# ZHKKKe/PixelSSL

Hardware: NVIDIA H100
Metric: images/sec DeepLab-v2-R101 MT 513x513 bs16 (higher is better)
Workload: dtype f16x3 (fp16 pairs, fp32 accumulate)

## Files before the change

include/pixelssl_b200.h:

```cpp
#ifndef PIXELSSL_B200_H
#define PIXELSSL_B200_H

#include <stdint.h>

#ifdef __cplusplus
extern "C" {
#endif

#define PXL_ERR_BAD_ARG   (-1)
#define PXL_ERR_UNSUPPORTED (-2)

int pxl_abi_version(void);
int64_t pxl_launch_count(void);
void pxl_reset_launch_count(void);

int64_t pxl_mse_workspace_bytes(void);
int pxl_mse_consistency(const float* s, const float* t, int64_t n, float loss_scale,
                        float* loss_out, float* grad_s, void* workspace, void* stream);
int pxl_mse_consistency_bwd(const float* s, const float* t, int64_t n, float loss_scale,
                            const float* upstream, float* grad_s, void* stream);

int pxl_ce2d(const float* logits, const float* labels, int n, int C, int64_t HW, int ignore_index,
             float* per_sample, float* grad_logits, const float* upstream, float upstream_const,
             void* stream);
// ... 69 lines not shown
} pxl_conv_geom;
#define PXL_MAX_TAPS 64
int pxl_conv_nhwc(const pxl_conv_geom* geom_host, const int* taps_dydx_host ,
                  const float* in, const float* w, const float* bias ,
                  float* out, void* stream);
int pxl_conv_wgrad_nhwc(const pxl_conv_geom* geom_host, const int* taps_dydx_host,
                        const float* in, const float* dy, float* dw, void* stream);
typedef struct {
    int w_ntaps;
    const int* widx_host;
    int out_mul, out_offy, out_offx, out_H, out_W;
    double* bn_stats;
    float out_scale;
    const float* out_scale_dev;
    int out_accumulate;
} pxl_conv_tc_ext;
int pxl_conv_tc_launch_ex(const pxl_conv_geom* geom_host, const int* taps_dydx_host, const pxl_conv_tc_ext* ext_host,
                          const float* in_hi, const float* in_lo, const float* w_hi, const float* w_lo,
                          const float* bias, float* out, void* stream);
int pxl_conv_wgrad_tc_launch(const pxl_conv_geom* geom_host, const int* taps_dydx_host, const float* in_hi,
                             const float* in_lo, const float* dy_hi, const float* dy_lo, float* dw,
                             void* stream);
int pxl_conv_h16_launch(const pxl_conv_geom* geom_host, const int* taps_dydx_host, const pxl_conv_tc_ext* ext_host,
                        const void* in_hi, const void* in_lo, const void* w_hi, const void* w_lo,
                        const float* bias, float* out, void* stream);
int pxl_conv_wgrad_h16_launch(const pxl_conv_geom* geom_host, const int* taps_dydx_host, const void* in_hi,
                              const void* in_lo, const void* dy_hi, const void* dy_lo, float* dw, float out_scale,
                              const float* out_scale_dev, void* stream);
int pxl_h16_split(const float* x, void* hi, void* lo, int64_t n, float scale, float* slot, int target_log2,
                  void* stream);
int pxl_h16_absmax(const float* x, int64_t n, float* slot, void* stream);
int pxl_h16_status(void);
int pxl_h16_status_sites(int* out4_host);
int pxl_h16_reset_status(void);
int pxl_split_tf32(const float* x, float* hi, float* lo, int64_t n, void* stream);
int pxl_conv_tc_status(void);
int pxl_conv_transpose_weights(const float* w, float* wt, int Cout, int T, int Cin, void* stream);
int pxl_conv_transpose_weights_batched(const float* src_base, float* dst_base, const int64_t* table, int n,
                                       int64_t total_tiles, void* stream);
int pxl_bias_grad(const float* dy, int64_t rows, int Cout, int ldo, float* dbias, int accumulate,
                  void* stream);

int pxl_stem_conv7x7s2(const float* img_planar, const float* w, float* out, int N, int H, int W,
                       int OH, int OW, void* stream);
int pxl_stem_conv7x7s2_wgrad(const float* img_planar, const float* dy, float* dw, int N, int H, int W,
                             int OH, int OW, void* stream);
int pxl_stem_im2col(const float* img_planar, float* cols, int N, int H, int W, int OH, int OW, void* stream);
int pxl_stem3x3s2_im2col(const float* img_planar, float* cols, int N, int H, int W, int OH, int OW, void* stream);

int pxl_sgd_ema(float* p, const float* g, float* buf, float* teacher, int64_t n, float lr,
                float momentum, float weight_decay, float ema_d, int first_step, void* stream);
// ... 102 lines not shown
```

pixelssl_b200/_lib.py:

```python
import ctypes
import os
import re

_HERE = os.path.dirname(os.path.abspath(__file__))
LIB_PATH = os.path.join(_HERE, 'lib', 'libpixelssl_b200.so')
HEADER_PATH = os.path.join(os.path.dirname(_HERE), 'include', 'pixelssl_b200.h')

c_void_p, c_int, c_int64, c_float, c_double = (ctypes.c_void_p, ctypes.c_int, ctypes.c_int64,
                                               ctypes.c_float, ctypes.c_double)
_SCALARS = {'int': c_int, 'int64_t': c_int64, 'float': c_float, 'double': c_double}


class ConvGeom(ctypes.Structure):
    _fields_ = [('N', c_int), ('H', c_int), ('W', c_int), ('Cin', c_int),
                ('OH', c_int), ('OW', c_int), ('Cout', c_int), ('ldo', c_int),
                ('mul', c_int), ('div', c_int), ('ntaps', c_int), ('precision', c_int)]


class ConvTcExt(ctypes.Structure):
    _fields_ = [('w_ntaps', c_int), ('widx_host', ctypes.POINTER(c_int)), ('out_mul', c_int),
                ('out_offy', c_int), ('out_offx', c_int), ('out_H', c_int), ('out_W', c_int),
                ('bn_stats', c_void_p), ('out_scale', c_float), ('out_scale_dev', c_void_p), ('out_accumulate', c_int)]


def header_code(path=HEADER_PATH):
    text = re.sub(r'/\*.*?\*/', ' ', open(path).read(), flags=re.S)
    return re.sub(r'^\s*#.*$', ' ', text, flags=re.M)


def ctype_of(decl, name, returned=False):
    if '*' in decl:
        return c_void_p
    words = [w for w in decl.split() if w != 'const']
    if returned and words == ['void']:
        return None
    t = ' '.join(words if returned else words[:-1])
    if t not in _SCALARS:
# ... 66 lines not shown
```

pixelssl_b200/csrc/common.cuh:

```cuda
#pragma once
#include <cuda_runtime.h>
#include <stdint.h>
#include "../../include/pixelssl_b200.h"

#define PXL_NUM_SMS 132

extern "C" void pxl_count_launch_(int n);
extern "C" int* pxl_h16_sat_counter(void);

#define PXL_WS_WGRAD 0
#define PXL_WS_BIAS 1
#define PXL_WS_CE 2
#define PXL_WS_CPS 3
#define PXL_WS_UNIMATCH 4
#define PXL_WS_STRONG_AUG 5
#define PXL_WS_OHEM 6
#define PXL_WS_DEPTHWISE 7
#define PXL_WS_PURPOSES 8
#define PXL_WS_STREAMS 8
extern "C" void* pxl_workspace_(int purpose, void* stream, size_t bytes, int* rc);

#define PXL_CHECK_LAUNCH()                                   \
    do {                                                     \
        pxl_count_launch_(1);                                \
        cudaError_t e__ = cudaPeekAtLastError();             \
        if (e__ != cudaSuccess) return (int)e__;             \
    } while (0)

static inline int64_t pxl_cdiv(int64_t a, int64_t b) { return (a + b - 1) / b; }

#define PXL_PDL_SYNC()                                                   \
    do {                                                                 \
        asm volatile("griddepcontrol.launch_dependents;" ::: "memory");  \
// ... 54 lines not shown
```

pixelssl_b200/csrc/conv_tc.cu:

```cuda
#include "common.cuh"
#include <cuda.h>
#include <cstdlib>
#include <type_traits>

typedef CUresult (*EncodeTiledFn)(CUtensorMap*, CUtensorMapDataType, cuuint32_t, void*, const cuuint64_t*,
                                  const cuuint64_t*, const cuuint32_t*, const cuuint32_t*, CUtensorMapInterleave,
                                  CUtensorMapSwizzle, CUtensorMapL2promotion, CUtensorMapFloatOOBfill);
static EncodeTiledFn get_encode() {
    static EncodeTiledFn fn = nullptr;
    if (!fn) {
        void* p = nullptr;
        cudaDriverEntryPointQueryResult q;
        if (cudaGetDriverEntryPoint("cuTensorMapEncodeTiled", &p, cudaEnableDefault, &q) == cudaSuccess &&
            q == cudaDriverEntryPointSuccess)
            fn = (EncodeTiledFn)p;
    }
    return fn;
}

static int make_act_map(CUtensorMap* m, const void* base, int C, int W, int H, int N, int bw, int bh, int estride = 1, int f16 = 0) {
    EncodeTiledFn enc = get_encode();
    if (!enc) return PXL_ERR_UNSUPPORTED;
    const cuuint64_t eb = f16 ? 2 : 4;
    cuuint64_t dims[4] = {(cuuint64_t)C, (cuuint64_t)W, (cuuint64_t)H, (cuuint64_t)N};
// ... 80 lines not shown
    uint64_t d = 0;
    d |= (uint64_t)((smem_addr & 0x3FFFF) >> 4);
    d |= (uint64_t)((lbo_bytes >> 4) & 0x3FFF) << 16;
    d |= (uint64_t)(1024 >> 4) << 32;
    d |= (uint64_t)1 << 62;
    return d;
}
__device__ __forceinline__ void wg_arrive() { asm volatile("wgmma.fence.sync.aligned;" ::: "memory"); }
__device__ __forceinline__ void wg_commit() { asm volatile("wgmma.commit_group.sync.aligned;" ::: "memory"); }
__device__ __forceinline__ void wg_wait0() { asm volatile("wgmma.wait_group.sync.aligned 0;" ::: "memory"); }
template <int R>
__device__ __forceinline__ void fence_regs(float (&d)[R]) {
#pragma unroll
    for (int i = 0; i < R; ++i) asm volatile("" : "+f"(d[i])::"memory");
}

template <int N, int KIND>
__device__ __forceinline__ void wgmma_op(float (&d)[N / 2], uint64_t da, uint64_t db, int scale_d);
template <> __device__ __forceinline__ void wgmma_op<32, 0>(float (&d)[16], uint64_t da, uint64_t db, int scale_d) {
    asm volatile(
        "{\n\t.reg .pred p;\n\tsetp.ne.b32 p, %18, 0;\n\t"
        "wgmma.mma_async.sync.aligned.m64n32k8.f32.tf32.tf32 {%0, %1, %2, %3, %4, %5, %6, %7, %8, %9, %10, %11, %12, %13, %14, %15}, %16, %17, p, 1, 1;\n\t}"
        : "+f"(d[0]), "+f"(d[1]), "+f"(d[2]), "+f"(d[3]), "+f"(d[4]), "+f"(d[5]), "+f"(d[6]), "+f"(d[7]), "+f"(d[8]), "+f"(d[9]), "+f"(d[10]), "+f"(d[11]), "+f"(d[12]), "+f"(d[13]), "+f"(d[14]), "+f"(d[15])
        : "l"(da), "l"(db), "r"(scale_d));
}
template <> __device__ __forceinline__ void wgmma_op<64, 0>(float (&d)[32], uint64_t da, uint64_t db, int scale_d) {
    asm volatile(
        "{\n\t.reg .pred p;\n\tsetp.ne.b32 p, %34, 0;\n\t"
        "wgmma.mma_async.sync.aligned.m64n64k8.f32.tf32.tf32 {%0, %1, %2, %3, %4, %5, %6, %7, %8, %9, %10, %11, %12, %13, %14, %15, %16, %17, %18, %19, %20, %21, %22, %23, %24, %25, %26, %27, %28, %29, %30, %31}, %32, %33, p, 1, 1;\n\t}"
        : "+f"(d[0]), "+f"(d[1]), "+f"(d[2]), "+f"(d[3]), "+f"(d[4]), "+f"(d[5]), "+f"(d[6]), "+f"(d[7]), "+f"(d[8]), "+f"(d[9]), "+f"(d[10]), "+f"(d[11]), "+f"(d[12]), "+f"(d[13]), "+f"(d[14]), "+f"(d[15]), "+f"(d[16]), "+f"(d[17]), "+f"(d[18]), "+f"(d[19]), "+f"(d[20]), "+f"(d[21]), "+f"(d[22]), "+f"(d[23]), "+f"(d[24]), "+f"(d[25]), "+f"(d[26]), "+f"(d[27]), "+f"(d[28]), "+f"(d[29]), "+f"(d[30]), "+f"(d[31])
// ... 69 lines not shown
    return h;
}

struct TcParams {
    int Cin, Cout, ldo, ntaps, kchunks;
    int N, OH, OW;
    int BW, BH, tilesW, tilesH;
    int stages, nsplit;
    int a_inkernel;
    int in_mul;
    int out_mul, out_offy, out_offx, outH, outW;
    int ntilesN, pix_tiles, total_tiles;
    int kc;
    float out_scale;
    int out_acc;
    short dy[PXL_MAX_TAPS], dx[PXL_MAX_TAPS], widx[PXL_MAX_TAPS];
};

#define TC_A_BYTES (128 * 128)
#define TC_MAX_STAGES 8
#define TC_THREADS 384

__device__ __forceinline__ void tc_tile_coords(const TcParams& p, int tile, int bn, int& n0, int& w0, int& h0, int& n) {
    const int nt = tile / p.pix_tiles, pix = tile - nt * p.pix_tiles;
    const int tw = pix % p.tilesW, th = (pix / p.tilesW) % p.tilesH;
    n = pix / (p.tilesW * p.tilesH);
    w0 = tw * p.BW; h0 = th * p.BH; n0 = nt * bn;
}

template <int BN, int F16>
__global__ void __launch_bounds__(TC_THREADS, 1)
conv_wg_kernel(const __grid_constant__ CUtensorMap mapA, const __grid_constant__ CUtensorMap mapAlo,
               const __grid_constant__ CUtensorMap mapB, const __grid_constant__ CUtensorMap mapBlo,
               const TcParams p, const float* __restrict__ bias, float* __restrict__ out,
               double* __restrict__ stats, int* __restrict__ err_flag, const float* __restrict__ oscale_ptr) {
    extern __shared__ __align__(1024) uint8_t smem_raw[];
    __shared__ uint64_t full_bar[TC_MAX_STAGES], empty_bar[TC_MAX_STAGES];
    __shared__ float st_warp[2][8][BN];

    uint8_t* smem = (uint8_t*)(((uintptr_t)smem_raw + 1023) & ~(uintptr_t)1023);
    constexpr int B_BYTES = BN * 128;
    constexpr int PER_OP = TC_A_BYTES + B_BYTES;
    const int stage_bytes = PER_OP * (p.nsplit == 3 ? 2 : 1);
    const int iters = p.ntaps * p.kchunks;

    if (threadIdx.x == 0) {
        for (int s = 0; s < p.stages; ++s) { mbar_init(&full_bar[s], 1); mbar_init(&empty_bar[s], 256); }
        asm volatile("fence.mbarrier_init.release.cluster;" ::: "memory");
    }
    __syncthreads();
    PXL_PDL_SYNC();

    if (threadIdx.x < 128) {
        asm volatile("setmaxnreg.dec.sync.aligned.u32 40;" ::: "memory");
        if (threadIdx.x >= 32) return;
        uint32_t tx = (uint32_t)((p.BW * p.BH * 128 + B_BYTES) * (p.nsplit == 3 ? 2 : 1));
        if (p.a_inkernel) tx -= (uint32_t)(p.BW * p.BH * 128);
        uint32_t s = 0, ph = 0;
        bool ok = true;
        for (int tile = blockIdx.x; tile < p.total_tiles && ok; tile += gridDim.x) {
            int n0, w0, h0, n;
            tc_tile_coords(p, tile, BN, n0, w0, h0, n);
            int tap = 0, c0 = 0;
            for (int it = 0; it < iters; ++it) {
                ok = __all_sync(0xffffffffu, mbar_wait(&empty_bar[s], ph ^ 1u, err_flag, 1));
                if (!ok) break;
                uint8_t* sa = smem + (size_t)s * stage_bytes;
                const int ax = w0 * p.in_mul + p.dx[tap], ay = h0 * p.in_mul + p.dy[tap];
                const int bk = p.widx[tap] * p.Cin + c0;
                if (elect_one()) {
                    mbar_expect_tx(&full_bar[s], tx);
                    tma_load_4d(sa, &mapA, &full_bar[s], c0, ax, ay, n);
                    tma_load_2d(sa + TC_A_BYTES, &mapB, &full_bar[s], bk, n0);
                    if (p.nsplit == 3) {
                        if (!p.a_inkernel) tma_load_4d(sa + PER_OP, &mapAlo, &full_bar[s], c0, ax, ay, n);
                        tma_load_2d(sa + PER_OP + TC_A_BYTES, &mapBlo, &full_bar[s], bk, n0);
                    }
                }
                __syncwarp();
                c0 += p.kc; if (c0 >= p.Cin) { c0 = 0; ++tap; }
                if (++s == (uint32_t)p.stages) { s = 0; ph ^= 1u; }
            }
        }
        return;
    }

    asm volatile("setmaxnreg.inc.sync.aligned.u32 232;" ::: "memory");
    const int ct = threadIdx.x - 128;
    const int cw = ct >> 7, t = ct & 127;
    const int warp = t >> 5, lane = t & 31;
    const float osc = p.out_scale * (oscale_ptr ? __ldg(oscale_ptr) : 1.f);
    const uint32_t smem_base = smem_u32(smem);
    const bool split3 = p.nsplit == 3;
    float acc[BN / 2], part[BN / 2], corr[BN / 2];
    uint32_t s = 0, ph = 0;
    int st_n0 = -1;
    float st_s = 0.f, st_q = 0.f;
    bool ok = true;
    auto flush_stats = [&]() {
        if (st_n0 >= 0 && ct < BN && st_n0 + ct < p.Cout && (st_s != 0.f || st_q != 0.f)) {
            atomicAdd(stats + st_n0 + ct, (double)st_s);
            atomicAdd(stats + p.Cout + st_n0 + ct, (double)st_q);
        }
        st_s = 0.f; st_q = 0.f;
    };
    auto f16_tile = [&](auto split3_c) -> bool {
        constexpr bool S3 = decltype(split3_c)::value;
        uint32_t prev = 0;
        for (int it = 0; it < iters; ++it) {
            if (!__all_sync(0xffffffffu, mbar_wait(&full_bar[s], ph, err_flag, 2))) { wg_wait0(); return false; }
            const uint32_t sa32 = smem_base + s * (uint32_t)stage_bytes;
            const uint32_t arow = (uint32_t)cw * (TC_A_BYTES / 2);
            const uint64_t da = sw128_desc(sa32 + arow), db = sw128_desc(sa32 + TC_A_BYTES);
            const uint64_t dal = sw128_desc(sa32 + PER_OP + arow), dbl = sw128_desc(sa32 + PER_OP + TC_A_BYTES);
            wg_arrive();
            fence_regs(part);
            if (S3) fence_regs(corr);
#pragma unroll
            for (int k = 0; k < 2; ++k) wgmma_op<BN, 1>(part, da + 2 * k, db + 2 * k, k);
            wg_commit();
            if (S3) {
#pragma unroll
                for (int k = 0; k < 4; ++k) wgmma_op<BN, 1>(corr, dal + 2 * k, db + 2 * k, k);
#pragma unroll
                for (int k = 0; k < 4; ++k) wgmma_op<BN, 1>(corr, da + 2 * k, dbl + 2 * k, 1);
                wg_commit();
                asm volatile("wgmma.wait_group.sync.aligned 1;" ::: "memory");
                fence_regs(part);
#pragma unroll
                for (int i = 0; i < BN / 2; ++i) acc[i] += part[i];
                wg_arrive();
                fence_regs(part);
#pragma unroll
                for (int k = 2; k < 4; ++k) wgmma_op<BN, 1>(part, da + 2 * k, db + 2 * k, k - 2);
                wg_commit();
                wg_wait0();
                fence_regs(part);
                fence_regs(corr);
                mbar_arrive(&empty_bar[s]);
#pragma unroll
                for (int i = 0; i < BN / 2; ++i) acc[i] += part[i] + corr[i];
            } else {
                asm volatile("wgmma.wait_group.sync.aligned 1;" ::: "memory");
                fence_regs(corr);
                if (it > 0) {
                    mbar_arrive(&empty_bar[prev]);
#pragma unroll
                    for (int i = 0; i < BN / 2; ++i) acc[i] += corr[i];
                }
                wg_arrive();
                fence_regs(corr);
#pragma unroll
                for (int k = 2; k < 4; ++k) wgmma_op<BN, 1>(corr, da + 2 * k, db + 2 * k, k - 2);
                wg_commit();
                asm volatile("wgmma.wait_group.sync.aligned 1;" ::: "memory");
                fence_regs(part);
#pragma unroll
                for (int i = 0; i < BN / 2; ++i) acc[i] += part[i];
            }
            prev = s;
            if (++s == (uint32_t)p.stages) { s = 0; ph ^= 1u; }
        }
        if (!S3) {
            wg_wait0();
            fence_regs(corr);
            mbar_arrive(&empty_bar[prev]);
#pragma unroll
            for (int i = 0; i < BN / 2; ++i) acc[i] += corr[i];
        }
        return true;
    };
    for (int tile = blockIdx.x; tile < p.total_tiles && ok; tile += gridDim.x) {
        int n0, w0, h0, n;
        tc_tile_coords(p, tile, BN, n0, w0, h0, n);
        if (stats && n0 != st_n0) { flush_stats(); st_n0 = n0; }
#pragma unroll
        for (int i = 0; i < BN / 2; ++i) acc[i] = 0.f;
        if constexpr (F16 != 0) ok = split3 ? f16_tile(std::true_type{}) : f16_tile(std::false_type{});
        else for (int it = 0; it < iters; ++it) {
            ok = __all_sync(0xffffffffu, mbar_wait(&full_bar[s], ph, err_flag, 2));
            if (!ok) break;
            uint8_t* sa = smem + (size_t)s * stage_bytes;
            if (p.a_inkernel) {
                float4* a_hi = reinterpret_cast<float4*>(sa + cw * (TC_A_BYTES / 2));
                float4* a_lo = reinterpret_cast<float4*>(sa + PER_OP + cw * (TC_A_BYTES / 2));
#pragma unroll
                for (int c = 0; c < TC_A_BYTES / 2 / 16 / 128; ++c) {
                    float4 lo;
                    const float4 hi = tf32_split4(a_hi[t + c * 128], lo);
                    a_hi[t + c * 128] = hi;
                    a_lo[t + c * 128] = lo;
                }
                fence_async_smem();
                named_bar(2 + cw, 128);
// ... 24 lines not shown
            for (int k = 2; k < 4; ++k) wgmma_op<BN, F16>(part, da + 2 * k, db + 2 * k, k - 2);
            wg_commit();
            wg_wait0();
            fence_regs(part);
            fence_regs(corr);
            mbar_arrive(&empty_bar[s]);
            if (split3) {
#pragma unroll
                for (int i = 0; i < BN / 2; ++i) acc[i] += part[i] + corr[i];
            } else {
#pragma unroll
                for (int i = 0; i < BN / 2; ++i) acc[i] += part[i];
            }
            if (++s == (uint32_t)p.stages) { s = 0; ph ^= 1u; }
        }
        if (!ok) break;
        int64_t obase[2];
        bool valid[2];
#pragma unroll
        for (int h = 0; h < 2; ++h) {
            const int r = cw * 64 + warp * 16 + (lane >> 2) + 8 * h;
            const int hy = r / p.BW, wx = r - hy * p.BW;
            const int oy = h0 + hy, ox = w0 + wx;
            valid[h] = hy < p.BH && oy < p.OH && ox < p.OW;
            obase[h] = ((int64_t)(n * p.outH + oy * p.out_mul + p.out_offy) * p.outW + ox * p.out_mul + p.out_offx) * p.ldo;
        }
        const bool vec2 = (p.ldo & 1) == 0 && ((uintptr_t)out & 7) == 0;
#pragma unroll
        for (int j = 0; j < BN / 8; ++j) {
            const int cl = j * 8 + 2 * (lane & 3);
            const int col = n0 + cl;
            const bool c0ok = col < p.Cout, c1ok = col + 1 < p.Cout;
            const float b0 = (bias && c0ok) ? __ldg(bias + col) : 0.f, b1 = (bias && c1ok) ? __ldg(bias + col + 1) : 0.f;
            float v[2][2];
#pragma unroll
            for (int h = 0; h < 2; ++h) {
                v[h][0] = acc[j * 4 + 2 * h] * osc + b0;
                v[h][1] = acc[j * 4 + 2 * h + 1] * osc + b1;
                if (!valid[h]) continue;
                float* o = out + obase[h] + col;
                if (p.out_acc) {
                    if (c0ok) o[0] += v[h][0];
                    if (c1ok) o[1] += v[h][1];
                } else if (c1ok && vec2) {
                    *reinterpret_cast<float2*>(o) = make_float2(v[h][0], v[h][1]);
                } else {
                    if (c0ok) o[0] = v[h][0];
// ... 5 lines not shown
                float s1 = (valid[0] ? v[0][1] : 0.f) + (valid[1] ? v[1][1] : 0.f);
                float q0 = (valid[0] ? v[0][0] * v[0][0] : 0.f) + (valid[1] ? v[1][0] * v[1][0] : 0.f);
                float q1 = (valid[0] ? v[0][1] * v[0][1] : 0.f) + (valid[1] ? v[1][1] * v[1][1] : 0.f);
#pragma unroll
                for (int o = 4; o < 32; o <<= 1) {
                    s0 += __shfl_xor_sync(0xffffffffu, s0, o); s1 += __shfl_xor_sync(0xffffffffu, s1, o);
                    q0 += __shfl_xor_sync(0xffffffffu, q0, o); q1 += __shfl_xor_sync(0xffffffffu, q1, o);
                }
                if (lane < 4) {
                    const int slot = cw * 4 + warp;
                    st_warp[0][slot][cl] = s0; st_warp[0][slot][cl + 1] = s1;
                    st_warp[1][slot][cl] = q0; st_warp[1][slot][cl + 1] = q1;
                }
            }
        }
        if (stats) {
            named_bar(1, 256);
            if (ct < BN) {
#pragma unroll
                for (int w8 = 0; w8 < 8; ++w8) { st_s += st_warp[0][w8][ct]; st_q += st_warp[1][w8][ct]; }
            }
            named_bar(1, 256);
        }
    }
    if (stats && ok) flush_stats();
}

__global__ void __launch_bounds__(256)
split_tf32_kernel(const float4* __restrict__ x, float4* __restrict__ hi, float4* __restrict__ lo, int64_t n4) {
    const int64_t stride = (int64_t)gridDim.x * blockDim.x;
    for (int64_t i = (int64_t)blockIdx.x * blockDim.x + threadIdx.x; i < n4; i += stride) {
        float4 l;
        hi[i] = tf32_split4(__ldcs(x + i), l);
        lo[i] = l;
    }
}

// ... 34 lines not shown
        int bh = 128 / bw;
        if (bh < 1) break;
        if (bh > 256) bh = 256;
        const int64_t tiles = (int64_t)((OW + bw - 1) / bw) * ((OH + bh - 1) / bh);
        const double eff = (double)OH * OW / ((double)tiles * 128.0);
        if (eff > best + 1e-9) { best = eff; BW = bw; BH = bh; }
    }
}

template <int BN, int F16>
static int fwd_smem_limit() {
    static const int v = query_dyn_smem_limit(conv_wg_kernel<BN, F16>);
    return v;
}

template <int BN, int F16>
static int launch_fwd(const CUtensorMap& mA, const CUtensorMap& mAlo, const CUtensorMap& mB, const CUtensorMap& mBlo,
                      const TcParams& p, size_t smem, cudaStream_t st, const float* bias, float* out, double* stats,
                      const float* oscale_ptr) {
    static bool attr = false;
    if (!attr) {
        cudaError_t e = cudaFuncSetAttribute(conv_wg_kernel<BN, F16>, cudaFuncAttributeMaxDynamicSharedMemorySize, fwd_smem_limit<BN, F16>());
        if (e != cudaSuccess) return (int)e;
        attr = true;
    }
    const unsigned nblk = (unsigned)(p.total_tiles < PXL_NUM_SMS ? p.total_tiles : PXL_NUM_SMS);
    cudaError_t le = pxl_launch_pdl(conv_wg_kernel<BN, F16>, dim3(nblk), dim3(TC_THREADS), smem, st, mA, mAlo, mB, mBlo, p,
                                    bias, out, stats, g_err_flag, oscale_ptr);
    if (le != cudaSuccess) return (int)le;
    PXL_CHECK_LAUNCH();
    return 0;
}

static int conv_tc_launch_core(const pxl_conv_geom* g, const int* taps, const pxl_conv_tc_ext* ext,
                               const void* in_hi, const void* in_lo, const void* w_hi, const void* w_lo,
                               const float* bias, float* out, void* stream);

extern "C" int pxl_conv_tc_launch_ex(const pxl_conv_geom* g, const int* taps, const pxl_conv_tc_ext* ext,
                                     const float* in_hi, const float* in_lo, const float* w_hi, const float* w_lo,
                                     const float* bias, float* out, void* stream) {
    if (g && g->precision > 2) return PXL_ERR_BAD_ARG;
    return conv_tc_launch_core(g, taps, ext, in_hi, in_lo, w_hi, w_lo, bias, out, stream);
}

extern "C" int pxl_conv_h16_launch(const pxl_conv_geom* g, const int* taps, const pxl_conv_tc_ext* ext,
                                   const void* in_hi, const void* in_lo, const void* w_hi, const void* w_lo,
                                   const float* bias, float* out, void* stream) {
    if (!g || (g->precision != 3 && g->precision != 4)) return PXL_ERR_BAD_ARG;
    return conv_tc_launch_core(g, taps, ext, in_hi, in_lo, w_hi, w_lo, bias, out, stream);
}

// ... 6 lines not shown
    const int kc = f16 ? 64 : 32;
    if (g->Cin % kc != 0 || g->ntaps > PXL_MAX_TAPS) return PXL_ERR_UNSUPPORTED;
    const int wtaps = ext && ext->w_ntaps > 0 ? ext->w_ntaps : g->ntaps;
    const int nsplit = (g->precision == 2 || g->precision == 3) ? 3 : 1;
    if (nsplit == 3 && !w_lo) return PXL_ERR_BAD_ARG;
    if (f16 && nsplit == 3 && !in_lo) return PXL_ERR_BAD_ARG;
    const int a_inkernel = (!f16 && nsplit == 3 && !in_lo) ? 1 : 0;
    const int omul = (ext && ext->out_mul > 0) ? ext->out_mul : 1;
    const bool has_out_xform = ext && (omul != 1 || ext->out_offy != 0 || ext->out_offx != 0);
    bool flat = (g->ntaps == 1 && taps[0] == 0 && taps[1] == 0 && g->OH == g->H && g->OW == g->W && g->mul == 1 &&
                 !has_out_xform);
    TcParams p;
    p.Cin = g->Cin; p.Cout = g->Cout; p.ldo = g->ldo; p.ntaps = g->ntaps; p.kchunks = g->Cin / kc;
    p.nsplit = nsplit; p.a_inkernel = a_inkernel; p.kc = kc;
    p.out_scale = (ext && ext->out_scale != 0.f) ? ext->out_scale : 1.f;
    const float* oscale_ptr = ext ? ext->out_scale_dev : nullptr;
    for (int t = 0; t < g->ntaps; ++t) {
        p.dy[t] = (short)taps[2 * t]; p.dx[t] = (short)taps[2 * t + 1];
        p.widx[t] = (short)((ext && ext->widx_host) ? ext->widx_host[t] : t);
        if (p.widx[t] < 0 || p.widx[t] >= wtaps) return PXL_ERR_BAD_ARG;
    }
    p.in_mul = g->mul;
    p.out_mul = omul; p.out_offy = has_out_xform ? ext->out_offy : 0; p.out_offx = has_out_xform ? ext->out_offx : 0;
    int mapW, mapH, mapN;
    if (flat) {
        const int64_t M = (int64_t)g->N * g->H * g->W;
        if (M >= (1ll << 31)) return PXL_ERR_UNSUPPORTED;
        p.N = 1; p.OH = 1; p.OW = (int)M;
        mapW = (int)M; mapH = 1; mapN = 1;
        p.outH = 1; p.outW = (int)M;
// ... 8 lines not shown
    const int stage_bytes = (TC_A_BYTES + BN * 128) * (nsplit == 3 ? 2 : 1);
    p.tilesW = (p.OW + p.BW - 1) / p.BW; p.tilesH = (p.OH + p.BH - 1) / p.BH;
    p.pix_tiles = p.N * p.tilesH * p.tilesW;
    p.ntilesN = (g->Cout + BN - 1) / BN;
    const int64_t n_tiles = (int64_t)p.pix_tiles * p.ntilesN;
    if (n_tiles >= (1ll << 31)) return PXL_ERR_UNSUPPORTED;
    p.total_tiles = (int)n_tiles;
    const int smem_limit = f16 ? (BN == 128 ? fwd_smem_limit<128, 1>() : BN == 64 ? fwd_smem_limit<64, 1>() : fwd_smem_limit<32, 1>())
                               : (BN == 128 ? fwd_smem_limit<128, 0>() : BN == 64 ? fwd_smem_limit<64, 0>() : fwd_smem_limit<32, 0>());
    if (smem_limit <= 0) return PXL_ERR_UNSUPPORTED;
    p.stages = (smem_limit - 1024) / stage_bytes;
    if (p.stages > TC_MAX_STAGES) p.stages = TC_MAX_STAGES;
    if (p.stages < 2) return PXL_ERR_UNSUPPORTED;
    const size_t smem = (size_t)p.stages * stage_bytes + 1024;

    CUtensorMap mA, mAlo, mB, mBlo;
    int rc = make_act_map(&mA, in_hi, g->Cin, mapW, mapH, mapN, p.BW, p.BH, g->mul, f16);
    if (rc) return rc;
    rc = make_w_map(&mB, w_hi, (int64_t)wtaps * g->Cin, g->Cout, BN, f16);
    if (rc) return rc;
    if (nsplit == 3) {
        if (a_inkernel) mAlo = mA;
        else {
            rc = make_act_map(&mAlo, in_lo, g->Cin, mapW, mapH, mapN, p.BW, p.BH, g->mul, f16);
            if (rc) return rc;
        }
        rc = make_w_map(&mBlo, w_lo, (int64_t)wtaps * g->Cin, g->Cout, BN, f16);
        if (rc) return rc;
    } else {
        mAlo = mA; mBlo = mB;
    }
    p.out_acc = (ext && ext->out_accumulate) ? 1 : 0;
    if ((rc = ensure_err_flag())) return rc;
    cudaStream_t st = (cudaStream_t)stream;
    double* st_ptr = ext ? (double*)ext->bn_stats : nullptr;
    if (f16) {
        if (BN == 128) return launch_fwd<128, 1>(mA, mAlo, mB, mBlo, p, smem, st, bias, out, st_ptr, oscale_ptr);
        if (BN == 64) return launch_fwd<64, 1>(mA, mAlo, mB, mBlo, p, smem, st, bias, out, st_ptr, oscale_ptr);
        return launch_fwd<32, 1>(mA, mAlo, mB, mBlo, p, smem, st, bias, out, st_ptr, oscale_ptr);
    }
    if (BN == 128) return launch_fwd<128, 0>(mA, mAlo, mB, mBlo, p, smem, st, bias, out, st_ptr, oscale_ptr);
    if (BN == 64) return launch_fwd<64, 0>(mA, mAlo, mB, mBlo, p, smem, st, bias, out, st_ptr, oscale_ptr);
    return launch_fwd<32, 0>(mA, mAlo, mB, mBlo, p, smem, st, bias, out, st_ptr, oscale_ptr);
}

extern "C" int pxl_conv_tc_status(void) {
    if (!g_err_flag) return 0;
    int v = 0;
    if (cudaMemcpy(&v, g_err_flag, sizeof(int), cudaMemcpyDeviceToHost) != cudaSuccess) return -1;
    return v;
}

extern "C" int pxl_conv_tc_impl(const pxl_conv_geom* g, const int* taps, const float* in, const float* w,
                                const float* bias, float* out, void* stream) {
    if (!g) return PXL_ERR_BAD_ARG;
    if (g->precision == 2) return PXL_ERR_UNSUPPORTED;
    if (g->precision > 2) return PXL_ERR_BAD_ARG;
    return conv_tc_launch_core(g, taps, nullptr, in, nullptr, w, nullptr, bias, out, stream);
// ... 405 lines not shown
```

pixelssl_b200/ops.py:

```python
import ctypes
import functools
import math

import torch

from . import _lib
from ._lib import ConvGeom, ConvTcExt, call
from .nn.peer import MAX_VALUES as _PEER_MAX_VALUES

CL = torch.channels_last
PRECISION = {'fp32': 0, 'tf32': 1, 'tf32x3': 2, 'f16x3': 3, 'f16': 4}
H16_FALLBACK = {3: 2, 4: 1}
H16_ACT_SCALE = 16.0
H16_W_SCALE = 256.0
H16_GRAD_TARGET_LOG2 = 14
_conv_precision = 0


def set_conv_precision(name):
    global _conv_precision
    _conv_precision = PRECISION[name]


def get_conv_precision():
    return _conv_precision


def _p(t):
    return t.data_ptr() if t is not None else None


# ... 630 lines not shown

def _stride2_dgrad_classes(taps, ntaps):
    classes = []
    for py in (0, 1):
        for px in (0, 1):
            sub, widx = [], []
            for t in range(ntaps):
                dy, dx = taps[2 * t], taps[2 * t + 1]
                if (py + dy) % 2 == 0 and (px + dx) % 2 == 0:
                    sub += [(py + dy) // 2, (px + dx) // 2]
                    widx.append(t)
            classes.append((py, px, sub, widx))
    return classes


def conv_raw(x, w_packed, bias, taps, N, H, W, Cin, OH, OW, Cout, ldo, mul, div, out=None, precision=None, bn_stats=None,
             accumulate=False):
    ntaps = len(taps) // 2
    family, prec = conv_route('fwd', Cin, Cout, mul, div, _conv_precision if precision is None else precision)
    if family != 'h16' and (isinstance(x, H16) or isinstance(w_packed, H16)):
        raise ValueError('fp16-pair operands given for a shape the f16 wgmma kernel does not cover')
    if out is None:
        out = torch.empty((N, ldo, OH, OW), dtype=torch.float32, device=(x[0] if isinstance(x, tuple) else x).device,
                          memory_format=CL)
        if ldo != Cout:
            out.zero_()
    if family == 'ffma':
        if isinstance(x, tuple):
            x = x[0] + x[1]
        if isinstance(w_packed, tuple):
            w_packed = w_packed[0] + w_packed[1]
        geom = ConvGeom(N, H, W, Cin, OH, OW, Cout, ldo, mul, div, ntaps, 0)
# ... 15 lines not shown
            ohs, ows = (OH - py + 1) // 2, (OW - px + 1) // 2
            if widx and ohs > 0 and ows > 0:
                launches.append((ConvGeom(N, H, W, Cin, ohs, ows, Cout, ldo, 1, 1, len(widx), prec), sub,
                                 ConvTcExt(ntaps, (ctypes.c_int * len(widx))(*widx), 2, py, px, OH, OW, None)))
    if family == 'h16':
        want_lo = prec == 3
        xh = x if isinstance(x, H16) else _pair_of(x, want_lo)
        wh = w_packed if isinstance(w_packed, H16) else conv_weight(w_packed, 'h16', (Cout, ntaps, Cin), want_lo=want_lo)
        fx, px = xh.inv_scale()
        fw, pw = wh.inv_scale()
        if px is not None and pw is not None:
            raise ValueError('at most one operand may carry a device-side scale')
        oscale, odev = fx * fw, _p(px if px is not None else pw)
        for geom, tp, ext in launches:
            ext.out_scale, ext.out_scale_dev, ext.out_accumulate = oscale, odev, 1 if accumulate else 0
            _timed_call('pxl_conv_h16_launch', ctypes.byref(geom), _ctaps(tp), ctypes.byref(ext), _p(xh.hi), _p(xh.lo),
                        _p(wh.hi), _p(wh.lo if want_lo else None), _p(bias), _p(out), _stream(),
                        meta=(2.0 * geom.N * geom.OH * geom.OW * geom.Cin * geom.Cout * geom.ntaps,
                              'fwd/dgrad N%d %dx%d Cin%d Cout%d taps%d mul%d' % (geom.N, geom.OH, geom.OW, geom.Cin, geom.Cout, geom.ntaps, geom.mul)))
        return out
    x_parts = x if isinstance(x, tuple) else (x, None)
    if prec == 2:
        w_parts = w_packed if isinstance(w_packed, tuple) else conv_weight(w_packed, 'split', (Cout, ntaps, Cin))
    else:
        w_parts = (w_packed, None)
    for geom, tp, ext in launches:
        _timed_call('pxl_conv_tc_launch_ex', ctypes.byref(geom), _ctaps(tp), ctypes.byref(ext) if ext is not None else None,
                    _p(x_parts[0]), _p(x_parts[1]), _p(w_parts[0]), _p(w_parts[1]), _p(bias), _p(out), _stream(),
                    meta=(2.0 * geom.N * geom.OH * geom.OW * geom.Cin * geom.Cout * geom.ntaps,
                          'fwd/dgrad(tf32) N%d %dx%d Cin%d Cout%d taps%d' % (geom.N, geom.OH, geom.OW, geom.Cin, geom.Cout, geom.ntaps)))
# ... 1345 lines not shown
```

Before: 166.6.

## Split last-wave conv tiles into narrower N sub-tiles to balance the tail

```diff
diff --git a/include/pixelssl_b200.h b/include/pixelssl_b200.h
--- a/include/pixelssl_b200.h
+++ b/include/pixelssl_b200.h
@@ -107,6 +107,7 @@
     float out_scale;
     const float* out_scale_dev;
     int out_accumulate;
+    int tail_split;
 } pxl_conv_tc_ext;
 int pxl_conv_tc_launch_ex(const pxl_conv_geom* geom_host, const int* taps_dydx_host, const pxl_conv_tc_ext* ext_host,
                           const float* in_hi, const float* in_lo, const float* w_hi, const float* w_lo,
@@ -128,6 +129,8 @@
 int pxl_h16_reset_status(void);
 int pxl_split_tf32(const float* x, float* hi, float* lo, int64_t n, void* stream);
 int pxl_conv_tc_status(void);
+int pxl_conv_tail_split(int tiles, int grid);
+int pxl_conv_tail_work(int tiles, int grid, int f, int cta, int* items_host, int max_items);
 int pxl_conv_transpose_weights(const float* w, float* wt, int Cout, int T, int Cin, void* stream);
 int pxl_conv_transpose_weights_batched(const float* src_base, float* dst_base, const int64_t* table, int n,
                                        int64_t total_tiles, void* stream);
diff --git a/pixelssl_b200/_lib.py b/pixelssl_b200/_lib.py
--- a/pixelssl_b200/_lib.py
+++ b/pixelssl_b200/_lib.py
@@ -20,7 +20,8 @@
 class ConvTcExt(ctypes.Structure):
     _fields_ = [('w_ntaps', c_int), ('widx_host', ctypes.POINTER(c_int)), ('out_mul', c_int),
                 ('out_offy', c_int), ('out_offx', c_int), ('out_H', c_int), ('out_W', c_int),
-                ('bn_stats', c_void_p), ('out_scale', c_float), ('out_scale_dev', c_void_p), ('out_accumulate', c_int)]
+                ('bn_stats', c_void_p), ('out_scale', c_float), ('out_scale_dev', c_void_p), ('out_accumulate', c_int),
+                ('tail_split', c_int)]
 
 
 def header_code(path=HEADER_PATH):
diff --git a/pixelssl_b200/csrc/common.cuh b/pixelssl_b200/csrc/common.cuh
--- a/pixelssl_b200/csrc/common.cuh
+++ b/pixelssl_b200/csrc/common.cuh
@@ -16,7 +16,8 @@
 #define PXL_WS_STRONG_AUG 5
 #define PXL_WS_OHEM 6
 #define PXL_WS_DEPTHWISE 7
-#define PXL_WS_PURPOSES 8
+#define PXL_WS_CONV_TAIL 8
+#define PXL_WS_PURPOSES 9
 #define PXL_WS_STREAMS 8
 extern "C" void* pxl_workspace_(int purpose, void* stream, size_t bytes, int* rc);
 
diff --git a/pixelssl_b200/csrc/conv_tc.cu b/pixelssl_b200/csrc/conv_tc.cu
--- a/pixelssl_b200/csrc/conv_tc.cu
+++ b/pixelssl_b200/csrc/conv_tc.cu
@@ -118,6 +118,11 @@
 #pragma unroll
     for (int i = 0; i < R; ++i) asm volatile("" : "+f"(d[i])::"memory");
 }
+template <int N, int R>
+__device__ __forceinline__ auto lead(float (&d)[R]) -> float (&)[N / 2] {
+    static_assert(N / 2 <= R, "narrower than the tile");
+    return *reinterpret_cast<float(*)[N / 2]>(&d[0]);
+}
 
 template <int N, int KIND>
 __device__ __forceinline__ void wgmma_op(float (&d)[N / 2], uint64_t da, uint64_t db, int scale_d);
@@ -217,6 +222,7 @@
     int kc;
     float out_scale;
     int out_acc;
+    int tail_f;
     short dy[PXL_MAX_TAPS], dx[PXL_MAX_TAPS], widx[PXL_MAX_TAPS];
 };
 
@@ -231,15 +237,67 @@
     w0 = tw * p.BW; h0 = th * p.BH; n0 = nt * bn;
 }
 
+__host__ __device__ __forceinline__ int tc_tail_start(int tiles, int grid) { return (tiles - 1) / grid * grid; }
+
+__host__ __device__ __forceinline__ int tc_sub_first(int m, int grid, int b) { return ((b - m) % grid + grid) % grid; }
+
+__host__ __device__ __forceinline__ bool tc_work(int tiles, int grid, int f, int bn, int b, int k, int& tile, int& coff,
+                                                 int& width) {
+    const int rec_end = f > 1 ? tc_tail_start(tiles, grid) : tiles;
+    const int nrec = b < rec_end ? (rec_end - 1 - b) / grid + 1 : 0;
+    coff = 0; width = bn;
+    if (k < nrec) { tile = b + k * grid; return true; }
+    if (f <= 1) return false;
+    const int m = tiles - rec_end;
+    const int s = tc_sub_first(m, grid, b) + (k - nrec) * grid;
+    if (s >= m * f) return false;
+    width = bn / f;
+    tile = rec_end + s / f; coff = (s % f) * width;
+    return true;
+}
+
+static const double kTailSubCost[3] = {1.0, 0.6, 0.55};
+
+extern "C" int pxl_conv_tail_split(int tiles, int grid) {
+    if (grid <= 0 || tiles <= grid) return 1;
+    const int r = (tiles + grid - 1) / grid, m = tiles - (r - 1) * grid;
+    int best_f = 1;
+    double best = 1.0;
+    for (int lf = 1; lf <= 2; ++lf) {
+        const int f = 1 << lf;
+        const double load = (double)((m * f + grid - 1) / grid) * kTailSubCost[lf];
+        if (load < best - 1e-9) { best = load; best_f = f; }
+    }
+    return best_f;
+}
+
+extern "C" int pxl_conv_tail_work(int tiles, int grid, int f, int cta, int* items_host, int max_items) {
+    if (tiles <= 0 || grid <= 0 || (f != 1 && f != 2 && f != 4) || cta < 0 || cta >= grid || (!items_host && max_items > 0))
+        return PXL_ERR_BAD_ARG;
+    int k = 0, tile, coff, width;
+    for (; tc_work(tiles, grid, f, 128, cta, k, tile, coff, width); ++k)
+        if (k < max_items) { items_host[3 * k] = tile; items_host[3 * k + 1] = coff; items_host[3 * k + 2] = width; }
+    return k;
+}
+
+#define TC_TAIL_SLOTS (2 * 8 * 128)
+#define TC_TAIL_TILE_FLOATS (TC_TAIL_SLOTS + 2 * 128)
+#define TC_TAIL_MAX PXL_NUM_SMS
+#define TC_TAIL_MIN_ITERS 16
+
 template <int BN, int F16>
 __global__ void __launch_bounds__(TC_THREADS, 1)
 conv_wg_kernel(const __grid_constant__ CUtensorMap mapA, const __grid_constant__ CUtensorMap mapAlo,
                const __grid_constant__ CUtensorMap mapB, const __grid_constant__ CUtensorMap mapBlo,
+               const __grid_constant__ CUtensorMap mapB64, const __grid_constant__ CUtensorMap mapBlo64,
+               const __grid_constant__ CUtensorMap mapB32, const __grid_constant__ CUtensorMap mapBlo32,
                const TcParams p, const float* __restrict__ bias, float* __restrict__ out,
-               double* __restrict__ stats, int* __restrict__ err_flag, const float* __restrict__ oscale_ptr) {
+               double* __restrict__ stats, int* __restrict__ err_flag, const float* __restrict__ oscale_ptr,
+               float* __restrict__ tail_ws, unsigned* __restrict__ tail_cnt) {
     extern __shared__ __align__(1024) uint8_t smem_raw[];
     __shared__ uint64_t full_bar[TC_MAX_STAGES], empty_bar[TC_MAX_STAGES];
     __shared__ float st_warp[2][8][BN];
+    __shared__ uint32_t tail_last;
 
     uint8_t* smem = (uint8_t*)(((uintptr_t)smem_raw + 1023) & ~(uintptr_t)1023);
     constexpr int B_BYTES = BN * 128;
@@ -261,9 +319,14 @@
         if (p.a_inkernel) tx -= (uint32_t)(p.BW * p.BH * 128);
         uint32_t s = 0, ph = 0;
         bool ok = true;
-        for (int tile = blockIdx.x; tile < p.total_tiles && ok; tile += gridDim.x) {
+        int tile, coff, width;
+        for (int k = 0; ok && tc_work(p.total_tiles, gridDim.x, p.tail_f, BN, blockIdx.x, k, tile, coff, width); ++k) {
             int n0, w0, h0, n;
             tc_tile_coords(p, tile, BN, n0, w0, h0, n);
+            n0 += coff;
+            const CUtensorMap* mb = width == BN ? &mapB : width == 64 ? &mapB64 : &mapB32;
+            const CUtensorMap* mbl = width == BN ? &mapBlo : width == 64 ? &mapBlo64 : &mapBlo32;
+            const uint32_t txk = tx - (uint32_t)((BN - width) * 128 * (p.nsplit == 3 ? 2 : 1));
             int tap = 0, c0 = 0;
             for (int it = 0; it < iters; ++it) {
                 ok = __all_sync(0xffffffffu, mbar_wait(&empty_bar[s], ph ^ 1u, err_flag, 1));
@@ -272,12 +335,12 @@
                 const int ax = w0 * p.in_mul + p.dx[tap], ay = h0 * p.in_mul + p.dy[tap];
                 const int bk = p.widx[tap] * p.Cin + c0;
                 if (elect_one()) {
-                    mbar_expect_tx(&full_bar[s], tx);
+                    mbar_expect_tx(&full_bar[s], txk);
                     tma_load_4d(sa, &mapA, &full_bar[s], c0, ax, ay, n);
-                    tma_load_2d(sa + TC_A_BYTES, &mapB, &full_bar[s], bk, n0);
+                    tma_load_2d(sa + TC_A_BYTES, mb, &full_bar[s], bk, n0);
                     if (p.nsplit == 3) {
                         if (!p.a_inkernel) tma_load_4d(sa + PER_OP, &mapAlo, &full_bar[s], c0, ax, ay, n);
-                        tma_load_2d(sa + PER_OP + TC_A_BYTES, &mapBlo, &full_bar[s], bk, n0);
+                        tma_load_2d(sa + PER_OP + TC_A_BYTES, mbl, &full_bar[s], bk, n0);
                     }
                 }
                 __syncwarp();
@@ -307,8 +370,12 @@
         }
         st_s = 0.f; st_q = 0.f;
     };
-    auto f16_tile = [&](auto split3_c) -> bool {
+    auto f16_tile = [&](auto split3_c, auto width_c) -> bool {
         constexpr bool S3 = decltype(split3_c)::value;
+        constexpr int NB = decltype(width_c)::value;
+        float (&pt)[NB / 2] = lead<NB>(part);
+        float (&cr)[NB / 2] = lead<NB>(corr);
+        float (&ac)[NB / 2] = lead<NB>(acc);
         uint32_t prev = 0;
         for (int it = 0; it < iters; ++it) {
             if (!__all_sync(0xffffffffu, mbar_wait(&full_bar[s], ph, err_flag, 2))) { wg_wait0(); return false; }
@@ -317,70 +384,119 @@
             const uint64_t da = sw128_desc(sa32 + arow), db = sw128_desc(sa32 + TC_A_BYTES);
             const uint64_t dal = sw128_desc(sa32 + PER_OP + arow), dbl = sw128_desc(sa32 + PER_OP + TC_A_BYTES);
             wg_arrive();
-            fence_regs(part);
-            if (S3) fence_regs(corr);
-#pragma unroll
-            for (int k = 0; k < 2; ++k) wgmma_op<BN, 1>(part, da + 2 * k, db + 2 * k, k);
+            fence_regs(pt);
+            if (S3) fence_regs(cr);
+#pragma unroll
+            for (int k = 0; k < 2; ++k) wgmma_op<NB, 1>(pt, da + 2 * k, db + 2 * k, k);
             wg_commit();
             if (S3) {
 #pragma unroll
-                for (int k = 0; k < 4; ++k) wgmma_op<BN, 1>(corr, dal + 2 * k, db + 2 * k, k);
-#pragma unroll
-                for (int k = 0; k < 4; ++k) wgmma_op<BN, 1>(corr, da + 2 * k, dbl + 2 * k, 1);
+                for (int k = 0; k < 4; ++k) wgmma_op<NB, 1>(cr, dal + 2 * k, db + 2 * k, k);
+#pragma unroll
+                for (int k = 0; k < 4; ++k) wgmma_op<NB, 1>(cr, da + 2 * k, dbl + 2 * k, 1);
                 wg_commit();
                 asm volatile("wgmma.wait_group.sync.aligned 1;" ::: "memory");
-                fence_regs(part);
-#pragma unroll
-                for (int i = 0; i < BN / 2; ++i) acc[i] += part[i];
+                fence_regs(pt);
+#pragma unroll
+                for (int i = 0; i < NB / 2; ++i) ac[i] += pt[i];
                 wg_arrive();
-                fence_regs(part);
-#pragma unroll
-                for (int k = 2; k < 4; ++k) wgmma_op<BN, 1>(part, da + 2 * k, db + 2 * k, k - 2);
+                fence_regs(pt);
+#pragma unroll
+                for (int k = 2; k < 4; ++k) wgmma_op<NB, 1>(pt, da + 2 * k, db + 2 * k, k - 2);
                 wg_commit();
                 wg_wait0();
-                fence_regs(part);
-                fence_regs(corr);
+                fence_regs(pt);
+                fence_regs(cr);
                 mbar_arrive(&empty_bar[s]);
 #pragma unroll
-                for (int i = 0; i < BN / 2; ++i) acc[i] += part[i] + corr[i];
+                for (int i = 0; i < NB / 2; ++i) ac[i] += pt[i] + cr[i];
             } else {
                 asm volatile("wgmma.wait_group.sync.aligned 1;" ::: "memory");
-                fence_regs(corr);
+                fence_regs(cr);
                 if (it > 0) {
                     mbar_arrive(&empty_bar[prev]);
 #pragma unroll
-                    for (int i = 0; i < BN / 2; ++i) acc[i] += corr[i];
+                    for (int i = 0; i < NB / 2; ++i) ac[i] += cr[i];
                 }
                 wg_arrive();
-                fence_regs(corr);
-#pragma unroll
-                for (int k = 2; k < 4; ++k) wgmma_op<BN, 1>(corr, da + 2 * k, db + 2 * k, k - 2);
+                fence_regs(cr);
+#pragma unroll
+                for (int k = 2; k < 4; ++k) wgmma_op<NB, 1>(cr, da + 2 * k, db + 2 * k, k - 2);
                 wg_commit();
                 asm volatile("wgmma.wait_group.sync.aligned 1;" ::: "memory");
-                fence_regs(part);
-#pragma unroll
-                for (int i = 0; i < BN / 2; ++i) acc[i] += part[i];
+                fence_regs(pt);
+#pragma unroll
+                for (int i = 0; i < NB / 2; ++i) ac[i] += pt[i];
             }
             prev = s;
             if (++s == (uint32_t)p.stages) { s = 0; ph ^= 1u; }
         }
         if (!S3) {
             wg_wait0();
-            fence_regs(corr);
+            fence_regs(cr);
             mbar_arrive(&empty_bar[prev]);
 #pragma unroll
-            for (int i = 0; i < BN / 2; ++i) acc[i] += corr[i];
+            for (int i = 0; i < NB / 2; ++i) ac[i] += cr[i];
         }
         return true;
     };
-    for (int tile = blockIdx.x; tile < p.total_tiles && ok; tile += gridDim.x) {
+    auto tail_arrive = [&](int ti, int q0, int nq) {
+        named_bar(1, 256);
+        if (ct == 0) {
+            uint32_t mask = 0;
+            for (int q = q0; q < q0 + nq; ++q) {
+                unsigned* c = tail_cnt + ti * 4 + q;
+                if (atomicAdd(c, 1u) == 1u) { mask |= 1u << q; atomicExch(c, 0u); }
+            }
+            __threadfence();
+            tail_last = mask;
+        }
+        named_bar(1, 256);
+        const uint32_t mask = tail_last;
+        if (ct < BN && ((mask >> (ct / (BN / p.tail_f))) & 1u)) {
+            const float* w = tail_ws + (size_t)ti * TC_TAIL_TILE_FLOATS;
+            float ss = __ldcg(w + TC_TAIL_SLOTS + ct), sq = __ldcg(w + TC_TAIL_SLOTS + 128 + ct);
+#pragma unroll
+            for (int w8 = 0; w8 < 8; ++w8) { ss += __ldcg(w + w8 * 128 + ct); sq += __ldcg(w + (8 + w8) * 128 + ct); }
+            int n0, w0, h0, n;
+            tc_tile_coords(p, tc_tail_start(p.total_tiles, gridDim.x) + ti, BN, n0, w0, h0, n);
+            if (ss != 0.f || sq != 0.f) {
+                atomicAdd(stats + n0 + ct, (double)ss);
+                atomicAdd(stats + p.Cout + n0 + ct, (double)sq);
+            }
+        }
+    };
+    auto tail_hand_off = [&]() {
+        const int m = p.total_tiles - tc_tail_start(p.total_tiles, gridDim.x);
+        if ((int)blockIdx.x >= m) return;
+        int n0, w0, h0, n;
+        tc_tile_coords(p, tc_tail_start(p.total_tiles, gridDim.x) + (int)blockIdx.x, BN, n0, w0, h0, n);
+        if (n0 != st_n0) { flush_stats(); st_n0 = n0; }
+        if (ct < BN) {
+            float* w = tail_ws + (size_t)blockIdx.x * TC_TAIL_TILE_FLOATS + TC_TAIL_SLOTS;
+            w[ct] = st_s; w[128 + ct] = st_q;
+            __threadfence();
+        }
+        st_s = 0.f; st_q = 0.f; st_n0 = -1;
+        tail_arrive(blockIdx.x, 0, p.tail_f);
+    };
+    auto tile_body = [&](auto sub_c, int tile, int coff, int width) -> bool {
+        constexpr bool sub = decltype(sub_c)::value;
+        bool ok = true;
         int n0, w0, h0, n;
         tc_tile_coords(p, tile, BN, n0, w0, h0, n);
-        if (stats && n0 != st_n0) { flush_stats(); st_n0 = n0; }
+        if (stats && !sub && n0 != st_n0) { flush_stats(); st_n0 = n0; }
 #pragma unroll
         for (int i = 0; i < BN / 2; ++i) acc[i] = 0.f;
-        if constexpr (F16 != 0) ok = split3 ? f16_tile(std::true_type{}) : f16_tile(std::false_type{});
-        else for (int it = 0; it < iters; ++it) {
+        if constexpr (F16 != 0 && BN == 128 && sub) {
+            using I64 = std::integral_constant<int, 64>;
+            using I32 = std::integral_constant<int, 32>;
+            if (width == 64) ok = split3 ? f16_tile(std::true_type{}, I64{}) : f16_tile(std::false_type{}, I64{});
+            else ok = split3 ? f16_tile(std::true_type{}, I32{}) : f16_tile(std::false_type{}, I32{});
+        } else if constexpr (F16 != 0) {
+            using IBN = std::integral_constant<int, BN>;
+            ok = split3 ? f16_tile(std::true_type{}, IBN{}) : f16_tile(std::false_type{}, IBN{});
+        } else for (int it = 0; it < iters; ++it) {
             ok = __all_sync(0xffffffffu, mbar_wait(&full_bar[s], ph, err_flag, 2));
             if (!ok) break;
             uint8_t* sa = smem + (size_t)s * stage_bytes;
@@ -435,7 +551,7 @@
             }
             if (++s == (uint32_t)p.stages) { s = 0; ph ^= 1u; }
         }
-        if (!ok) break;
+        if (!ok) return false;
         int64_t obase[2];
         bool valid[2];
 #pragma unroll
@@ -450,8 +566,8 @@
 #pragma unroll
         for (int j = 0; j < BN / 8; ++j) {
             const int cl = j * 8 + 2 * (lane & 3);
-            const int col = n0 + cl;
-            const bool c0ok = col < p.Cout, c1ok = col + 1 < p.Cout;
+            const int col = n0 + coff + cl;
+            const bool c0ok = col < p.Cout && cl < width, c1ok = col + 1 < p.Cout && cl + 1 < width;
             const float b0 = (bias && c0ok) ? __ldg(bias + col) : 0.f, b1 = (bias && c1ok) ? __ldg(bias + col + 1) : 0.f;
             float v[2][2];
 #pragma unroll
@@ -487,13 +603,34 @@
                 }
             }
         }
-        if (stats) {
+        if (stats && !sub) {
             named_bar(1, 256);
             if (ct < BN) {
 #pragma unroll
                 for (int w8 = 0; w8 < 8; ++w8) { st_s += st_warp[0][w8][ct]; st_q += st_warp[1][w8][ct]; }
             }
             named_bar(1, 256);
+        } else if (stats) {
+            named_bar(1, 256);
+            const int ti = tile - tc_tail_start(p.total_tiles, gridDim.x);
+            if (ct < width) {
+                float* w = tail_ws + (size_t)ti * TC_TAIL_TILE_FLOATS + coff + ct;
+#pragma unroll
+                for (int w8 = 0; w8 < 8; ++w8) { w[w8 * 128] = st_warp[0][w8][ct]; w[(8 + w8) * 128] = st_warp[1][w8][ct]; }
+                __threadfence();
+            }
+            tail_arrive(ti, coff / width, 1);
+        }
+        return true;
+    };
+    const int rec_end = p.tail_f > 1 ? tc_tail_start(p.total_tiles, gridDim.x) : p.total_tiles;
+    for (int tile = blockIdx.x; tile < rec_end && ok; tile += gridDim.x) ok = tile_body(std::false_type{}, tile, 0, BN);
+    if constexpr (F16 != 0 && BN == 128) {
+        if (p.tail_f > 1 && ok) {
+            if (stats) tail_hand_off();
+            const int m = p.total_tiles - rec_end, wd = BN / p.tail_f;
+            for (int sidx = tc_sub_first(m, gridDim.x, blockIdx.x); sidx < m * p.tail_f && ok; sidx += gridDim.x)
+                ok = tile_body(std::true_type{}, rec_end + sidx / p.tail_f, (sidx % p.tail_f) * wd, wd);
         }
     }
     if (stats && ok) flush_stats();
@@ -558,10 +695,12 @@
     return v;
 }
 
+struct TcWeightMaps { CUtensorMap b, blo, b64, blo64, b32, blo32; };
+
 template <int BN, int F16>
-static int launch_fwd(const CUtensorMap& mA, const CUtensorMap& mAlo, const CUtensorMap& mB, const CUtensorMap& mBlo,
+static int launch_fwd(const CUtensorMap& mA, const CUtensorMap& mAlo, const TcWeightMaps& wm,
                       const TcParams& p, size_t smem, cudaStream_t st, const float* bias, float* out, double* stats,
-                      const float* oscale_ptr) {
+                      const float* oscale_ptr, float* tail_ws, unsigned* tail_cnt) {
     static bool attr = false;
     if (!attr) {
         cudaError_t e = cudaFuncSetAttribute(conv_wg_kernel<BN, F16>, cudaFuncAttributeMaxDynamicSharedMemorySize, fwd_smem_limit<BN, F16>());
@@ -569,8 +708,9 @@
         attr = true;
     }
     const unsigned nblk = (unsigned)(p.total_tiles < PXL_NUM_SMS ? p.total_tiles : PXL_NUM_SMS);
-    cudaError_t le = pxl_launch_pdl(conv_wg_kernel<BN, F16>, dim3(nblk), dim3(TC_THREADS), smem, st, mA, mAlo, mB, mBlo, p,
-                                    bias, out, stats, g_err_flag, oscale_ptr);
+    cudaError_t le = pxl_launch_pdl(conv_wg_kernel<BN, F16>, dim3(nblk), dim3(TC_THREADS), smem, st, mA, mAlo, wm.b, wm.blo,
+                                    wm.b64, wm.blo64, wm.b32, wm.blo32, p, bias, out, stats, g_err_flag, oscale_ptr,
+                                    tail_ws, tail_cnt);
     if (le != cudaSuccess) return (int)le;
     PXL_CHECK_LAUNCH();
     return 0;
@@ -579,6 +719,26 @@
 static int conv_tc_launch_core(const pxl_conv_geom* g, const int* taps, const pxl_conv_tc_ext* ext,
                                const void* in_hi, const void* in_lo, const void* w_hi, const void* w_lo,
                                const float* bias, float* out, void* stream);
+
+static int tail_workspace(cudaStream_t st, float** ws, unsigned** cnt) {
+    const size_t fbytes = (size_t)TC_TAIL_MAX * TC_TAIL_TILE_FLOATS * sizeof(float);
+    const size_t cbytes = (size_t)TC_TAIL_MAX * 4 * sizeof(unsigned);
+    int rc = 0;
+    uint8_t* buf = (uint8_t*)pxl_workspace_(PXL_WS_CONV_TAIL, st, fbytes + cbytes, &rc);
+    if (rc) return rc;
+    static const void* zeroed[PXL_WS_STREAMS];
+    int i = 0;
+    while (i < PXL_WS_STREAMS && zeroed[i] && zeroed[i] != buf) ++i;
+    if (i == PXL_WS_STREAMS) return PXL_ERR_UNSUPPORTED;
+    if (!zeroed[i]) {
+        cudaError_t e = cudaMemsetAsync(buf + fbytes, 0, cbytes, st);
+        if (e != cudaSuccess) return (int)e;
+        zeroed[i] = buf;
+    }
+    *ws = (float*)buf;
+    *cnt = (unsigned*)(buf + fbytes);
+    return 0;
+}
 
 extern "C" int pxl_conv_tc_launch_ex(const pxl_conv_geom* g, const int* taps, const pxl_conv_tc_ext* ext,
                                      const float* in_hi, const float* in_lo, const float* w_hi, const float* w_lo,
@@ -615,6 +775,7 @@
     p.Cin = g->Cin; p.Cout = g->Cout; p.ldo = g->ldo; p.ntaps = g->ntaps; p.kchunks = g->Cin / kc;
     p.nsplit = nsplit; p.a_inkernel = a_inkernel; p.kc = kc;
     p.out_scale = (ext && ext->out_scale != 0.f) ? ext->out_scale : 1.f;
+    p.tail_f = 1;
     const float* oscale_ptr = ext ? ext->out_scale_dev : nullptr;
     for (int t = 0; t < g->ntaps; ++t) {
         p.dy[t] = (short)taps[2 * t]; p.dx[t] = (short)taps[2 * t + 1];
@@ -653,10 +814,16 @@
     if (p.stages < 2) return PXL_ERR_UNSUPPORTED;
     const size_t smem = (size_t)p.stages * stage_bytes + 1024;
 
-    CUtensorMap mA, mAlo, mB, mBlo;
+    const int grid = p.total_tiles < PXL_NUM_SMS ? p.total_tiles : PXL_NUM_SMS;
+    p.tail_f = (ext && ext->tail_split && f16 && BN == 128 && g->Cout % 128 == 0 && p.ntaps * p.kchunks >= TC_TAIL_MIN_ITERS)
+                   ? pxl_conv_tail_split(p.total_tiles, grid) : 1;
+
+    CUtensorMap mA, mAlo;
+    TcWeightMaps wm;
+    const int64_t wK = (int64_t)wtaps * g->Cin;
     int rc = make_act_map(&mA, in_hi, g->Cin, mapW, mapH, mapN, p.BW, p.BH, g->mul, f16);
     if (rc) return rc;
-    rc = make_w_map(&mB, w_hi, (int64_t)wtaps * g->Cin, g->Cout, BN, f16);
+    rc = make_w_map(&wm.b, w_hi, wK, g->Cout, BN, f16);
     if (rc) return rc;
     if (nsplit == 3) {
         if (a_inkernel) mAlo = mA;
@@ -664,23 +831,35 @@
             rc = make_act_map(&mAlo, in_lo, g->Cin, mapW, mapH, mapN, p.BW, p.BH, g->mul, f16);
             if (rc) return rc;
         }
-        rc = make_w_map(&mBlo, w_lo, (int64_t)wtaps * g->Cin, g->Cout, BN, f16);
+        rc = make_w_map(&wm.blo, w_lo, wK, g->Cout, BN, f16);
         if (rc) return rc;
     } else {
-        mAlo = mA; mBlo = mB;
+        mAlo = mA; wm.blo = wm.b;
+    }
+    wm.b64 = wm.b32 = wm.b; wm.blo64 = wm.blo32 = wm.blo;
+    if (p.tail_f > 1) {
+        const int sub_w = BN / p.tail_f;
+        CUtensorMap* hi = sub_w == 64 ? &wm.b64 : &wm.b32;
+        CUtensorMap* lo = sub_w == 64 ? &wm.blo64 : &wm.blo32;
+        if ((rc = make_w_map(hi, w_hi, wK, g->Cout, sub_w, f16))) return rc;
+        if (nsplit == 3) { if ((rc = make_w_map(lo, w_lo, wK, g->Cout, sub_w, f16))) return rc; }
+        else *lo = *hi;
     }
     p.out_acc = (ext && ext->out_accumulate) ? 1 : 0;
     if ((rc = ensure_err_flag())) return rc;
     cudaStream_t st = (cudaStream_t)stream;
     double* st_ptr = ext ? (double*)ext->bn_stats : nullptr;
+    float* tail_ws = nullptr;
+    unsigned* tail_cnt = nullptr;
+    if (p.tail_f > 1 && st_ptr && (rc = tail_workspace(st, &tail_ws, &tail_cnt))) return rc;
     if (f16) {
-        if (BN == 128) return launch_fwd<128, 1>(mA, mAlo, mB, mBlo, p, smem, st, bias, out, st_ptr, oscale_ptr);
-        if (BN == 64) return launch_fwd<64, 1>(mA, mAlo, mB, mBlo, p, smem, st, bias, out, st_ptr, oscale_ptr);
-        return launch_fwd<32, 1>(mA, mAlo, mB, mBlo, p, smem, st, bias, out, st_ptr, oscale_ptr);
-    }
-    if (BN == 128) return launch_fwd<128, 0>(mA, mAlo, mB, mBlo, p, smem, st, bias, out, st_ptr, oscale_ptr);
-    if (BN == 64) return launch_fwd<64, 0>(mA, mAlo, mB, mBlo, p, smem, st, bias, out, st_ptr, oscale_ptr);
-    return launch_fwd<32, 0>(mA, mAlo, mB, mBlo, p, smem, st, bias, out, st_ptr, oscale_ptr);
+        if (BN == 128) return launch_fwd<128, 1>(mA, mAlo, wm, p, smem, st, bias, out, st_ptr, oscale_ptr, tail_ws, tail_cnt);
+        if (BN == 64) return launch_fwd<64, 1>(mA, mAlo, wm, p, smem, st, bias, out, st_ptr, oscale_ptr, tail_ws, tail_cnt);
+        return launch_fwd<32, 1>(mA, mAlo, wm, p, smem, st, bias, out, st_ptr, oscale_ptr, tail_ws, tail_cnt);
+    }
+    if (BN == 128) return launch_fwd<128, 0>(mA, mAlo, wm, p, smem, st, bias, out, st_ptr, oscale_ptr, tail_ws, tail_cnt);
+    if (BN == 64) return launch_fwd<64, 0>(mA, mAlo, wm, p, smem, st, bias, out, st_ptr, oscale_ptr, tail_ws, tail_cnt);
+    return launch_fwd<32, 0>(mA, mAlo, wm, p, smem, st, bias, out, st_ptr, oscale_ptr, tail_ws, tail_cnt);
 }
 
 extern "C" int pxl_conv_tc_status(void) {
diff --git a/pixelssl_b200/ops.py b/pixelssl_b200/ops.py
--- a/pixelssl_b200/ops.py
+++ b/pixelssl_b200/ops.py
@@ -1,6 +1,7 @@
 import ctypes
 import functools
 import math
+import os
 
 import torch
 
@@ -15,6 +16,7 @@
 H16_W_SCALE = 256.0
 H16_GRAD_TARGET_LOG2 = 14
 _conv_precision = 0
+CONV_TAIL = os.environ.get('PXL_CONV_TAIL', '1') != '0'
 
 
 def set_conv_precision(name):
@@ -675,8 +677,22 @@
     return classes
 
 
+def conv_tail_split(tiles, grid):
+    return int(_lib.load().pxl_conv_tail_split(tiles, grid))
+
+
+def conv_tail_work(tiles, grid, f, cta):
+    n = int(_lib.load().pxl_conv_tail_work(tiles, grid, f, cta, None, 0))
+    if n < 0:
+        raise ValueError('pxl_conv_tail_work: bad arguments')
+    buf = (ctypes.c_int * (3 * max(n, 1)))()
+    call_count = int(_lib.load().pxl_conv_tail_work(tiles, grid, f, cta, buf, n))
+    assert call_count == n
+    return [tuple(buf[3 * i:3 * i + 3]) for i in range(n)]
+
+
 def conv_raw(x, w_packed, bias, taps, N, H, W, Cin, OH, OW, Cout, ldo, mul, div, out=None, precision=None, bn_stats=None,
-             accumulate=False):
+             accumulate=False, tail=None):
     ntaps = len(taps) // 2
     family, prec = conv_route('fwd', Cin, Cout, mul, div, _conv_precision if precision is None else precision)
     if family != 'h16' and (isinstance(x, H16) or isinstance(w_packed, H16)):
@@ -722,6 +738,7 @@
         oscale, odev = fx * fw, _p(px if px is not None else pw)
         for geom, tp, ext in launches:
             ext.out_scale, ext.out_scale_dev, ext.out_accumulate = oscale, odev, 1 if accumulate else 0
+            ext.tail_split = 1 if (CONV_TAIL if tail is None else tail) else 0
             _timed_call('pxl_conv_h16_launch', ctypes.byref(geom), _ctaps(tp), ctypes.byref(ext), _p(xh.hi), _p(xh.lo),
                         _p(wh.hi), _p(wh.lo if want_lo else None), _p(bias), _p(out), _stream(),
                         meta=(2.0 * geom.N * geom.OH * geom.OW * geom.Cin * geom.Cout * geom.ntaps,
```

Measured after the change: 169.3, median of 6. 1.6% higher.
